# georghess/neurad-studio

Hardware: NVIDIA H100
Metric: rays/sec (camera+lidar) (higher is better)
Workload: dtype f32

## Files before the change

### neurad-studio_b200/csrc/b200nerf.cu

```cuda
#include <cuda_runtime.h>

#include <cstdio>
#include <cstring>
#include <new>
#include <string>
#include <vector>

#include "../../include/b200nerf.h"
#include "nff_device.h"
#include "nff_lane.h"
#include "rgb_decoder.cuh"
#include "modules.cuh"

using namespace nff;

static thread_local std::string g_err;
static int fail(int code, const std::string& msg) {
  g_err = msg;
  return code;
}
#define CUDA_TRY(expr)                                                                                   \
  do {                                                                                                   \
    cudaError_t e_ = (expr);                                                                             \
    if (e_ != cudaSuccess)                                                                               \
// ... 56 lines not shown
    if (prev != dev) cudaSetDevice(dev);
  }
  ~DeviceGuard() { cudaSetDevice(prev); }
};

int make_grid(const b200nerf_grid_desc* d, const float* table, Grid* g) {
  REQUIRE(d != nullptr, "grid descriptor is NULL");
  REQUIRE(d->num_levels >= 1 && d->num_levels <= kMaxLevels, "num_levels must be in [1,16]");
  REQUIRE(d->log2_hashmap_size >= 1 && d->log2_hashmap_size <= 30, "log2_hashmap_size out of range");
  g->table = table;
  g->T = 1u << d->log2_hashmap_size;
  g->mask = g->T - 1u;
  g->L = d->num_levels;
  g->F = d->features_per_level;
  for (int i = 0; i < kMaxLevels; ++i) g->res[i] = i < d->num_levels ? d->scalings[i] : 0.f;
  return 0;
}
}

#ifndef NFF_WARPS
#define NFF_WARPS 8
#endif
constexpr int kSmemMaxOptIn = 227 * 1024;
constexpr int kRenderWarps = NFF_WARPS;

template <int WARPS>
__global__ void __launch_bounds__(WARPS * 32, 16 / WARPS) nff_render_kernel(const __grid_constant__ RenderParams P) {
  extern __shared__ __align__(16) unsigned char smem_raw[];
  float* mlp_s = reinterpret_cast<float*>(smem_raw);
  constexpr int kMlpBytes = (kMainMlpFloats * 4 + 15) / 16 * 16;
// ... 60 lines not shown
  *ray_out = active ? ray : fallback;
  return active;
}

__device__ __forceinline__ int64_t lane_patches(const RenderParams& P) {
  return P.rays.image_width > 0 ? lane_units(P) * (kLaneThreads / 32) : (P.n_rays + 31) / 32;
}
__device__ __forceinline__ bool lane_patch_ray(const RenderParams& P, int64_t patch, int lane_, int64_t* ray_out) {
  constexpr int kPatchesPerUnit = kLaneThreads / 32;
  return lane_unit_ray(P, patch / kPatchesPerUnit, (int)(patch % kPatchesPerUnit) * 32 + lane_, ray_out);
}

#ifndef NFF_SAMPLE_CTAS
#define NFF_SAMPLE_CTAS 2
#endif
template <int LAYOUT>
__global__ void __launch_bounds__(kLaneThreads, NFF_SAMPLE_CTAS) nff_sample_lane_kernel(const __grid_constant__ RenderParams P,
                                                                                        float* __restrict__ scratch,
                                                                                        float* __restrict__ handoff) {
  const int tid = threadIdx.x, warp = __shfl_sync(0xffffffffu, (int)(threadIdx.x >> 5), 0), lane_ = tid & 31;
  const LaneScratch sc = lane_scratch_of(scratch, blockIdx.x);
  constexpr int kPPU = kLaneThreads / 32;
  const int64_t n_patches = lane_patches(P);
  const int64_t full_rounds = n_patches / kPPU / gridDim.x;
  const int64_t r0 = full_rounds * gridDim.x * kPPU, rest = n_patches - r0;
  const int64_t p0 = r0 + rest * blockIdx.x / gridDim.x, p1 = r0 + rest * (blockIdx.x + 1) / gridDim.x;
  for (int64_t it = 0;; ++it) {
    int64_t patch;
    if (it < full_rounds) {
      patch = (it * gridDim.x + blockIdx.x) * kPPU + warp;
    } else {
      patch = p0 + warp + (it - full_rounds) * kPPU;
      if (patch >= p1) break;
    }
    int64_t ray;
    const bool active = lane_patch_ray(P, patch, lane_, &ray);
    const LaneRay R = lane_ray_setup(P, sc, tid, ray);
    float* col = active ? handoff + ray : sc.bins2 + tid;
    sample_ray_lane<LAYOUT>(P, sc, R, tid, ray, active, col, active ? P.n_rays : (int64_t)kLaneThreads);
  }
}

template <int LAYOUT>
__global__ void __launch_bounds__(kLaneThreads, kLaneCtasPerSm) nff_shade_lane_kernel(const __grid_constant__ RenderParams P,
                                                                                      float* __restrict__ scratch,
                                                                                      const float* __restrict__ handoff) {
  extern __shared__ __align__(128) unsigned char smem_shade[];
  TcShared* tcs = reinterpret_cast<TcShared*>(smem_shade);
  const int tid = threadIdx.x, warp = __shfl_sync(0xffffffffu, (int)(threadIdx.x >> 5), 0), group = warp >> 2;
  tc_stage_weights(*tcs, P.main_mlp_nn, tid, kLaneThreads, true);
  tc::fence_async_smem();
  __syncthreads();
  MlpLaneTc mlp;
  mlp.t = tcs;
// ... 711 lines not shown
  c->sm_count = prop.multiProcessorCount;
  CUDA_TRY(cudaFuncSetAttribute(nff_render_kernel<kRenderWarps>, cudaFuncAttributeMaxDynamicSharedMemorySize,
                                (int)((kMainMlpFloats * 4 + 15) / 16 * 16 + kRenderWarps * sizeof(WarpShared))));
  CUDA_TRY(cudaFuncSetAttribute(nff_render_tc_kernel<kRenderWarps>, cudaFuncAttributeMaxDynamicSharedMemorySize,
                                (int)(tc_smem_bytes(kRenderWarps * 32) + kRenderWarps * sizeof(WarpSharedTc))));
  CUDA_TRY(cudaMalloc((void**)&c->d_status, sizeof(int)));
  CUDA_TRY(cudaMemset(c->d_status, 0, sizeof(int)));
  CUDA_TRY(cudaFuncSetAttribute(nff_render_lane_kernel, cudaFuncAttributeMaxDynamicSharedMemorySize,
                                (int)lane_tc_smem_bytes()));
  c->lane_ctas = c->sm_count * (kLaneCtasPerSm > NFF_SAMPLE_CTAS ? kLaneCtasPerSm : NFF_SAMPLE_CTAS);
  CUDA_TRY(cudaMalloc((void**)&c->d_lane_scratch, sizeof(float) * lane_scratch_floats_per_cta() * c->lane_ctas));
  CUDA_TRY(cudaFuncSetAttribute(nff_shade_lane_kernel<0>, cudaFuncAttributeMaxDynamicSharedMemorySize,
                                (int)lane_tc_smem_bytes()));
  CUDA_TRY(cudaFuncSetAttribute(nff_shade_lane_kernel<1>, cudaFuncAttributeMaxDynamicSharedMemorySize,
                                (int)lane_tc_smem_bytes()));
  CUDA_TRY(cudaFuncSetAttribute(nff_sample_lane_kernel<0>, cudaFuncAttributePreferredSharedMemoryCarveout, 0));
  CUDA_TRY(cudaFuncSetAttribute(nff_sample_lane_kernel<1>, cudaFuncAttributePreferredSharedMemoryCarveout, 0));
  CUDA_TRY(cudaMalloc((void**)&c->d_minmax, 2 * sizeof(unsigned)));
  c->handoff_rays = (int64_t)1 << 21;
  CUDA_TRY(cudaMalloc((void**)&c->d_handoff, sizeof(float) * (kS2 + 1) * c->handoff_rays));
  CUDA_TRY(cudaMalloc((void**)&c->d_grad_actor_ptrs, sizeof(float*) * kModMaxActors));
  *out = c;
  return 0;
}

int b200nerf_destroy(b200nerf_ctx* c) {
  if (!c) return 0;
  DeviceGuard g(c->device);
  for (int i = 0; i < 3; ++i) {
    cudaFree((void*)c->d_actor_tables[i]);
    cudaFree(c->d_decoder[i]);
  }
// ... 36 lines not shown
    return fail(B200NERF_ERR_UNSUPPORTED,
                "fused kernel is specialised for NeuRAD's grid shapes (main: 8 levels x 4 features, proposal: 6 x 1)");
  if (n_actors > 0) {
    REQUIRE(ad && atabs_host, "actor grid descriptor / tables missing");
    if (int e = make_grid(ad, nullptr, &fg.act)) return e;
    if (fg.act.L != 4 || fg.act.F != wantF)
      return fail(B200NERF_ERR_UNSUPPORTED, "actor grids must have 4 levels and the static grid's feature width");
    cudaFree((void*)c->d_actor_tables[field]);
    c->d_actor_tables[field] = nullptr;
    CUDA_TRY(cudaMalloc((void**)&c->d_actor_tables[field], sizeof(float*) * n_actors));
    CUDA_TRY(cudaMemcpy((void*)c->d_actor_tables[field], atabs_host, sizeof(float*) * n_actors, cudaMemcpyHostToDevice));
    fg.actor_tables = c->d_actor_tables[field];
  }
  fg.static_scale = static_scale;
  fg.actor_scale = actor_scale;
  fg.decoder = c->d_decoder[field];
  c->fields[field] = fg;
  c->have_field[field] = true;
  c->field_layout[field] = 0;
  if (field == B200NERF_FIELD_MAIN) c->layout = 0;
  return 0;
}

namespace {
int make_tcnn_grid(const b200nerf_tcnn_grid_desc* d, const float* params, int want_dims, Grid* g) {
  REQUIRE(d != nullptr && params != nullptr, "tcnn grid descriptor / parameters are NULL");
  REQUIRE(d->num_levels >= 1 && d->num_levels <= kMaxLevels, "num_levels must be in [1,16]");
  REQUIRE(d->n_input_dims == want_dims, "tcnn grid has the wrong number of input dimensions (static: 3, actors: 4)");
  *g = Grid{};
  g->table = params;
// ... 26 lines not shown
  DeviceGuard g(c->device);
  FieldGrids fg{};
  if (int e = make_tcnn_grid(sd, sparams, 3, &fg.stat)) return e;
  const int wantL = field == B200NERF_FIELD_MAIN ? 8 : 6, wantF = field == B200NERF_FIELD_MAIN ? 4 : 1;
  if (fg.stat.L != wantL || fg.stat.F != wantF)
    return fail(B200NERF_ERR_UNSUPPORTED,
                "fused kernel is specialised for NeuRAD's grid shapes (main: 8 levels x 4 features, proposal: 6 x 1)");
  if (n_actors > 0) {
    if (int e = make_tcnn_grid(ad, aparams, 4, &fg.act)) return e;
    if (fg.act.L != 4 || fg.act.F != wantF)
      return fail(B200NERF_ERR_UNSUPPORTED, "the 4-D actor grid must have 4 levels and the static grid's feature width");
  }
  fg.n_actors_f = (float)(n_actors > 0 ? n_actors : 1);
  fg.static_scale = static_scale;
  fg.actor_scale = actor_scale;
  fg.decoder = c->d_decoder[field];
  c->fields[field] = fg;
  c->have_field[field] = true;
  c->field_layout[field] = 1;
  if (field == B200NERF_FIELD_MAIN) c->layout = 1;
  return 0;
}

int b200nerf_set_proposal_decoder(b200nerf_ctx* c, int field, const float* weight, int in_dim) {
  REQUIRE(c, "ctx is NULL");
  REQUIRE(field == B200NERF_FIELD_PROP0 || field == B200NERF_FIELD_PROP1, "decoder belongs to a proposal field");
  REQUIRE(weight && in_dim == 6, "density_decoder must be Linear(6, 1)");
  DeviceGuard g(c->device);
  if (!c->d_decoder[field]) CUDA_TRY(cudaMalloc((void**)&c->d_decoder[field], sizeof(float) * 8));
  CUDA_TRY(cudaMemcpyAsync(c->d_decoder[field], weight, sizeof(float) * in_dim, cudaMemcpyDeviceToDevice, c->param_stream));
// ... 117 lines not shown
            "density_field_of_round entries must name a proposal field");
  DeviceGuard g(c->device);
  if (!c->d_u1) CUDA_TRY(cudaMalloc((void**)&c->d_u1, sizeof(float) * (kS1 + 1)));
  if (!c->d_u2) CUDA_TRY(cudaMalloc((void**)&c->d_u2, sizeof(float) * (kS2 + 1)));
  CUDA_TRY(cudaMemcpy(c->d_u1, u1_host, sizeof(float) * (kS1 + 1), cudaMemcpyHostToDevice));
  CUDA_TRY(cudaMemcpy(c->d_u2, u2_host, sizeof(float) * (kS2 + 1), cudaMemcpyHostToDevice));
  Sampling s{};
  s.lam = lam;
  s.scaling = scaling;
  s.sky_distance = sky;
  s.hist_pad = hist_pad;
  s.cam_area_scale = camera_area_scale;
  double lam1 = lam - 1.0 < 0 ? -(lam - 1.0) : (lam - 1.0);
  s.lam_1 = (float)lam1;
  s.ratio = (float)(lam1 / (double)lam);
  s.u1 = c->d_u1;
  s.u2 = c->d_u2;
  s.field_of_round[0] = field_of_round[0];
  s.field_of_round[1] = field_of_round[1];
  c->samp = s;
  c->n_prop0 = n_prop0; c->n_prop1 = n_prop1; c->n_nerf = n_nerf;
  c->have_samp = true;
  return 0;
}

int b200nerf_nff_render_fwd(b200nerf_ctx* c, const b200nerf_rays* rays, int64_t n_rays, const b200nerf_outputs* out,
                            const b200nerf_trace* trace, void* stream) {
  REQUIRE(c && rays && out, "NULL argument");
  REQUIRE(n_rays >= 0, "negative ray count");
  REQUIRE(rays->image_width >= 0, "negative image_width");
// ... 61 lines not shown
    }
    const int fdim = kNff + c->app.dim;
    for (int64_t start = 0; start < n_rays; start += slice) {
      const int64_t cnt = n_rays - start < slice ? n_rays - start : slice;
      RenderParams Q = P;
      Q.n_rays = cnt;
      offset_rays(Q, start, fdim);
      int64_t need = (cnt + kLaneThreads - 1) / kLaneThreads;
      if (rays->image_width > 0) {
        const int64_t W = rays->image_width, H = (cnt + W - 1) / W;
        need = ((W + 31) / 32) * ((H + kLaneThreads / 32 - 1) / (kLaneThreads / 32));
      }
      const int64_t max_a = (int64_t)c->sm_count * NFF_SAMPLE_CTAS, max_b = (int64_t)c->sm_count * kLaneCtasPerSm;
      const int64_t patches = rays->image_width > 0 ? need * (kLaneThreads / 32) : (cnt + 31) / 32, groups = (patches + 3) / 4;
      const int64_t grid_a = patches < max_a ? patches : max_a, grid_b = groups < max_b ? groups : max_b;
      if (c->layout == 1) {
        nff_sample_lane_kernel<1><<<(int)grid_a, kLaneThreads, 0, st>>>(Q, c->d_lane_scratch, c->d_handoff);
        nff_shade_lane_kernel<1><<<(int)grid_b, kLaneThreads, smem, st>>>(Q, c->d_lane_scratch, c->d_handoff);
      } else {
        nff_sample_lane_kernel<0><<<(int)grid_a, kLaneThreads, 0, st>>>(Q, c->d_lane_scratch, c->d_handoff);
        nff_shade_lane_kernel<0><<<(int)grid_b, kLaneThreads, smem, st>>>(Q, c->d_lane_scratch, c->d_handoff);
      }
    }
  } else if (c->mlp_mode == 2) {
    const size_t smem = lane_tc_smem_bytes();
    int64_t need = (n_rays + kLaneThreads - 1) / kLaneThreads;
    if (rays->image_width > 0) {
      const int64_t W = rays->image_width, H = (n_rays + W - 1) / W;
      need = ((W + 31) / 32) * ((H + kLaneThreads / 32 - 1) / (kLaneThreads / 32));
    }
    int lane_blocks = (int)(need < c->lane_ctas ? need : c->lane_ctas);
    nff_render_lane_kernel<<<lane_blocks, kLaneThreads, smem, st>>>(P, c->d_lane_scratch);
  } else if (c->mlp_mode == 1) {
    const size_t smem = tc_smem_bytes(WARPS * 32) + WARPS * sizeof(WarpSharedTc);
    nff_render_tc_kernel<WARPS><<<blocks, WARPS * 32, smem, st>>>(P);
// ... 83 lines not shown
  CUDA_TRY(cudaGetLastError());
  return 0;
}

static int make_spacing(int kind, float power_lambda, float power_scaling, SpacingArgs* a) {
  REQUIRE(kind >= B200NERF_SPACING_UNIFORM && kind <= B200NERF_SPACING_LOG, "unknown spacing kind");
  a->kind = kind;
  if (kind == B200NERF_SPACING_POWER) {
    REQUIRE(power_lambda != 0.f && power_lambda != 1.f, "power_lambda 0 / 1 (log / identity spacing) is not supported");
    REQUIRE(power_scaling > 0.f, "power_scaling must be positive");
    a->power.lam = power_lambda;
    a->power.scaling = power_scaling;
    double lam1 = power_lambda - 1.0 < 0 ? -(power_lambda - 1.0) : (power_lambda - 1.0);
    a->power.lam_1 = (float)lam1;
    a->power.ratio = (float)(lam1 / (double)power_lambda);
  }
  return 0;
}

int b200nerf_spaced_sample(b200nerf_ctx* c, int kind, float power_lambda, float power_scaling, const float* nears,
                           const float* fars, int64_t n_rays, int n_samples, float* bins_s, float* bins_e, void* stream) {
  REQUIRE(c, "ctx is NULL");
  REQUIRE(n_rays >= 0 && n_samples >= 1, "bad sample grid");
  if (n_rays == 0) return 0;
  REQUIRE(fars && bins_e, "NULL argument");
  SpacingArgs a{};
  if (int rc = make_spacing(kind, power_lambda, power_scaling, &a)) return rc;
  DeviceGuard g(c->device);
  const int64_t n = n_rays * (n_samples + 1);
  spaced_sample_kernel<<<(unsigned)((n + 255) / 256), 256, 0, (cudaStream_t)stream>>>(a, nears, fars, n_rays, n_samples, bins_s, bins_e);
// ... 801 lines not shown
```

### neurad-studio_b200/csrc/nff_device.h

```cpp
#pragma once
#include "nff_params.h"
#include "simt.h"

#ifndef NFF_G_PROP
#define NFF_G_PROP 1
#endif
#ifndef NFF_G_ACT
#define NFF_G_ACT 2
#endif
#ifndef NFF_ILP
#define NFF_ILP 2
#endif
#ifndef NFF_F4_UNROLL
#define NFF_F4_UNROLL 2
#endif
#ifndef NFF_FAST_RCP
#define NFF_FAST_RCP 1
#endif
#ifndef NFF_PARITY_STD
#define NFF_PARITY_STD 0
#endif
#ifndef NFF_PARITY_LERP
#define NFF_PARITY_LERP 0
#endif
// ... 20 lines not shown
  for (int d = 1; d < 32; d <<= 1) {
    float n = shfl_up(v, d);
    if (lane() >= d) v += n;
  }
  return v;
}
NFF_D float warp_scan_mul(float v) {
#pragma unroll
  for (int d = 1; d < 32; d <<= 1) {
    float n = shfl_up(v, d);
    if (lane() >= d) v *= n;
  }
  return v;
}

NFF_D float pow_lam(float t, float e) { return e == -1.0f ? frcp(t) : powf(t, e); }
NFF_D float spacing_fn(float x, const Sampling& s) {
  float t = fadd(fdiv(fmul(x, s.scaling), s.lam_1), 1.0f);
  return fmul(s.ratio, fsub(pow_lam(t, s.lam), 1.0f));
}
NFF_D float spacing_fn_inv(float y, const Sampling& s) {
  float t = fadd(fdiv(fmul(y, s.lam), s.lam_1), 1.0f);
  t = fmaxf(t, 1e-10f);
  float r = fmul(fsub(pow_lam(t, s.lam == -1.0f ? -1.0f : 1.0f / s.lam), 1.0f), s.lam_1);
  return fdiv(r, s.scaling);
}
NFF_D float to_euclid(float u, float s_near, float s_far, const Sampling& s) {
  return spacing_fn_inv(fadd(fmul(u, s_far), fmul(fsub(1.0f, u), s_near)), s);
}
NFF_D float linspace01(int i, int n) {
  float step = fdiv(1.0f, (float)n);
  return i < (n + 1) / 2 ? fmul(step, (float)i) : fsub(1.0f, fmul(step, (float)(n - i)));
}

struct Gauss {
  float x, y, z, std;
};
NFF_D Gauss sample_gaussian(const float o[3], const float d[3], float area, float start, float end) {
  float md = fdiv(fsub(end, start), 2.0f);
  float t = fadd(start, md);
  Gauss g;
  g.x = fadd(o[0], fmul(d[0], t));
  g.y = fadd(o[1], fmul(d[1], t));
  g.z = fadd(o[2], fmul(d[2], t));
  float cs = fmul(area, fmul(t, t));
#if NFF_PARITY_STD
  g.std = powf(fmul(cs, md), 0.33333334f);
#else
  g.std = cbrtf(fmul(cs, md));
#endif
  return g;
}
NFF_D Gauss contract(Gauss g, float scale) {
  float x = fdiv(g.x, scale), y = fdiv(g.y, scale), z = fdiv(g.z, scale);
#if NFF_PARITY_STD
  float sd = fdiv(g.std, scale);
#else
  float sd = fmul(g.std, frcp(scale));
#endif
  float mag = fmaxf(fmaxf(fabsf(x), fabsf(y)), fabsf(z));
  if (!(mag < 1.0f)) {
    const float a = fsub(2.0f, frcp(mag));
    x = fmul(a, fdiv(x, mag));
    y = fmul(a, fdiv(y, mag));
    z = fmul(a, fdiv(z, mag));
#if NFF_PARITY_STD
    float q = fdiv(powf(fsub(fmul(2.0f, mag), 1.0f), 0.33333334f), mag);
#else
    float q = fmul(cbrtf(fsub(fmul(2.0f, mag), 1.0f)), frcp(mag));
#endif
    sd = fmul(sd, fmul(q, q));
  }
  Gauss r;
  r.x = fmul(fadd(x, 2.0f), 0.25f);
  r.y = fmul(fadd(y, 2.0f), 0.25f);
  r.z = fmul(fadd(z, 2.0f), 0.25f);
  r.std = fmul(sd, 0.25f);
  return r;
}

struct Cell {
  uint32_t hx[2], hy[2], hz[2];
  float ox, oy, oz;
};
NFF_D Cell grid_cell(float x, float y, float z, float res) {
  float px = fmul(x, res), py = fmul(y, res), pz = fmul(z, res);
  float fx = floorf(px), fy = floorf(py), fz = floorf(pz);
  Cell c;
  const uint32_t ix = (uint32_t)(int32_t)fx, iy = (uint32_t)(int32_t)fy, iz = (uint32_t)(int32_t)fz;
  c.hx[0] = ix;
  c.hx[1] = ix + (px != fx ? 1u : 0u);
  c.hy[0] = iy * 2654435761u;
  c.hy[1] = (iy + (py != fy ? 1u : 0u)) * 2654435761u;
// ... 57 lines not shown
  float ox, oy, oz;
};
template <int SH>
NFF_D CellB<SH> grid_cell_b(float x, float y, float z, float res) {
  const float px = fmul(x, res), py = fmul(y, res), pz = fmul(z, res);
  const float fx = floorf(px), fy = floorf(py), fz = floorf(pz);
  CellB<SH> c;
  c.hx = (uint32_t)(int32_t)fx << SH;
  c.hy = (uint32_t)(int32_t)fy * (2654435761u << SH);
  c.hz = (uint32_t)(int32_t)fz * (805459861u << SH);
  c.ox = fsub(px, fx);
  c.oy = fsub(py, fy);
  c.oz = fsub(pz, fz);
  return c;
}
NFF_D uint32_t xor_and(uint32_t a, uint32_t b, uint32_t m) {
#if defined(__CUDACC__)
  uint32_t d;
  asm("lop3.b32 %0, %1, %2, %3, 0x28;" : "=r"(d) : "r"(a), "r"(b), "r"(m));
  return d;
#else
  return (a ^ b) & m;
#endif
}
template <int SH>
NFF_D void cell_offsets_b(const CellB<SH>& c, uint32_t maskb, uint32_t r[8]) {
  const uint32_t hx1 = c.hx + (1u << SH), hy1 = c.hy + (2654435761u << SH), hz1 = c.hz + (805459861u << SH);
  const uint32_t a11 = hy1 ^ hz1, a01 = c.hy ^ hz1, a10 = hy1 ^ c.hz, a00 = c.hy ^ c.hz;
  r[0] = xor_and(hx1, a11, maskb);
  r[1] = xor_and(hx1, a01, maskb);
// ... 31 lines not shown
  float f4756 = blend_f(f47, c.oy, f56, iy);
  return blend_f(f0312, c.oz, f4756, iz);
}

template <int L, int G>
NFF_D float encode_f1_dot(const float* NFF_RESTRICT table, const Grid& gr, Gauss g, const float* NFF_RESTRICT dec) {
  static_assert(L % G == 0, "group size must divide the level count");
  float acc = 0.0f;
  const uint32_t maskb = gr.mask << 2;
#pragma unroll
  for (int l0 = 0; l0 < L; l0 += G) {
    CellB<2> c[G];
    float f[G][8];
#pragma unroll
    for (int j = 0; j < G; ++j) {
      c[j] = grid_cell_b<2>(g.x, g.y, g.z, gr.res[l0 + j]);
      uint32_t r[8];
      cell_offsets_b<2>(c[j], maskb, r);
      const char* base = level_base(table, l0 + j, gr.T, 4);
#pragma unroll
      for (int k = 0; k < 8; ++k) f[j][k] = ldg_at<float>(base, r[k]);
    }
#pragma unroll
    for (int j = 0; j < G; ++j) {
      float w = level_weight(gr.res[l0 + j], g.std);
      float v = trilerp_b<2>(f[j], c[j], 1.0f - c[j].ox, 1.0f - c[j].oy, 1.0f - c[j].oz);
      acc = fmaf(fmul(v, w), ldg(dec + l0 + j), acc);
    }
  }
  return acc;
}
// ... 685 lines not shown
```

### neurad-studio_b200/csrc/nff_lane.h

```cpp
#pragma once
#include "nff_device.h"

namespace nff {

#ifndef NFF_LANE_THREADS
#define NFF_LANE_THREADS 512
#endif
#ifndef NFF_F4_WEIGHTS
#define NFF_F4_WEIGHTS 0
#endif
constexpr int kLaneThreads = NFF_LANE_THREADS;
constexpr int kLaneCtasPerSm = 512 / kLaneThreads;
constexpr int kCandFloats = 16;
constexpr int kLaneMaxCand = 32;

struct LaneScratch {
  float* w;
  float* bins1;
  float* bins2;
  float* cand;
};
NFF_HD size_t lane_scratch_floats_per_cta() {
  return (size_t)kLaneThreads * (kS0 + (kS1 + 1) + (kS2 + 1) + kLaneMaxCand * kCandFloats);
}
// ... 81 lines not shown
#pragma unroll
      for (int i = 0; i < 12; ++i) M_out[i] = M[i];
    }
  }
  return hit;
}

template <int LAYOUT = 0>
NFF_D float lane_proposal_density(const FieldGrids& fg, const LaneScratch& sc, int tid, int n_cand, const Gauss& g,
                                  int* actor_id) {
  float pb[3], M[12];
  int a = n_cand > 0 ? lane_actor_of_sample(sc, tid, n_cand, g, pb, M) : -1;
  float acc;
  if (a >= 0) {
    Gauss ga = {pb[0], pb[1], pb[2], g.std};
    ga = contract(ga, fg.actor_scale);
    if (LAYOUT == 1) {
      const float x4[4] = {ga.x, ga.y, ga.z, fdiv((float)a, fg.n_actors_f)};
      acc = tcnn_encode_f1_dot<4>(fg.act, 4, x4, ga.std, fg.decoder);
    } else {
      acc = encode_f1_dot<4, NFF_G_ACT>(fg.actor_tables[a], fg.act, ga, fg.decoder);
    }
  } else {
    Gauss gs = contract(g, fg.static_scale);
    if (LAYOUT == 1) {
      const float x3[3] = {gs.x, gs.y, gs.z};
      acc = tcnn_encode_f1_dot<3>(fg.stat, 6, x3, gs.std, fg.decoder);
    } else {
      acc = encode_f1_dot<6, NFF_G_PROP>(fg.stat.table, fg.stat, gs, fg.decoder);
    }
  }
  *actor_id = a;
  return expf(acc);
}

NFF_D void encode_f4_col(const float* NFF_RESTRICT table, const Grid& gr, int L, Gauss g, float* x , int pitch) {
  const uint32_t maskb = gr.mask << 4;
#pragma unroll 2
  for (int l = 0; l < L; ++l) {
// ... 40 lines not shown
#endif
  }
}

struct LaneRoundIO {
  int S, S_new;
  const float* u_tab;
  float* bins_out;
  int64_t bins_stride;
  float* tr_w;
  int32_t* tr_aid;
  float* tr_bins_s;
  float* tr_bins_e;
  int32_t* tr_inds;
};
template <int LAYOUT = 0>
NFF_D float lane_proposal_round(const RenderParams& P, const FieldGrids& fg, const LaneScratch& sc, int tid, int n_cand,
                                const LaneRoundIO& io, const float* bins_in, const float o[3], const float d[3], float area,
                                float s_near, float s_far, int64_t ray) {
  const Sampling& sp = P.samp;
  const int S = io.S, S_new = io.S_new;
  auto edge = [bins_in, S](int i) { return bins_in ? bins_in[(size_t)i * kLaneThreads] : linspace01(i, S); };
  double excl = 0.0, tot_d = 0.0;
  float depth_acc = 0.0f;
  float e_prev = to_euclid(edge(0), s_near, s_far, sp);
#pragma unroll 1
  for (int s = 0; s < S; ++s) {
    const float T = expf(-(float)excl);
    float w = 0.0f;
    if (!(vote_all_converged(T == 0.0f) && io.tr_aid == nullptr)) {
      const float e0 = e_prev;
      const float e1 = to_euclid(edge(s + 1), s_near, s_far, sp);
      e_prev = e1;
      Gauss g = sample_gaussian(o, d, area, e0, e1);
      int aid;
      float dens = lane_proposal_density<LAYOUT>(fg, sc, tid, n_cand, g, &aid);
      float dd = fmul(fsub(e1, e0), dens);
      float alpha = fsub(1.0f, expf(-dd));
      excl += (double)dd;
      w = nan_to_num(fmul(alpha, T));
      depth_acc = fadd(depth_acc, fmul(w, fmul(fadd(e0, e1), 0.5f)));
      if (io.tr_aid) io.tr_aid[ray * S + s] = aid;
    }
    if (io.tr_w) io.tr_w[ray * S + s] = w;
    w = fadd(w, sp.hist_pad);
    sc.w[(size_t)s * kLaneThreads + tid] = w;
    tot_d += (double)w;
  }
  float tot = (float)tot_d;
  const float padding = fmaxf(fsub(1e-5f, tot), 0.0f);
  const float pad_each = fdiv(padding, (float)S);
  tot = fadd(tot, padding);
  int k = 1;
  double run = (double)fdiv(fadd(sc.w[tid], pad_each), tot);
  float c_km1 = 0.0f, c_k = fminf(1.0f, (float)run);
  float w_next = sc.w[(size_t)kLaneThreads + tid];
#pragma unroll 1
  for (int i = 0; i <= S_new; ++i) {
    const float u = ldg(io.u_tab + i);
    while (k <= S && c_k <= u) {
      ++k;
      c_km1 = c_k;
      if (k <= S) {
        const float wk = w_next;
        w_next = sc.w[(size_t)(k < S ? k : S - 1) * kLaneThreads + tid];
        run += (double)fdiv(fadd(wk, pad_each), tot);
        c_k = fminf(1.0f, (float)run);
      }
    }
    const int above = k > S ? S : k;
    const float b0 = edge(k - 1), b1 = edge(above);
    float t = nan_to_num(fdiv(fsub(u, c_km1), fsub(k > S ? c_km1 : c_k, c_km1)));
    t = fminf(fmaxf(t, 0.0f), 1.0f);
    const float nb = fadd(b0, fmul(t, fsub(b1, b0)));
    io.bins_out[(size_t)i * io.bins_stride] = nb;
    if (io.tr_inds) io.tr_inds[ray * (S_new + 1) + i] = k;
    if (io.tr_bins_s) io.tr_bins_s[ray * (S_new + 1) + i] = nb;
    if (io.tr_bins_e) io.tr_bins_e[ray * (S_new + 1) + i] = to_euclid(nb, s_near, s_far, sp);
  }
  return depth_acc;
}

struct MlpLaneFfma {
  static constexpr int kPitch = kLaneThreads;
  const float* w;
  float* panel_;
  int sh_tcnn = 0;
  NFF_D float* panel() const { return panel_; }
  NFF_D void run(const float* x, const float dir[3], float& sdf, float* feat, int ) const {
    float h[kHidden], go[kNff + 1], in2[kNff + kSh], h2[kHidden];
    dense<kGeoIn, kHidden, kHidden, true>(w + kOffGeoW0, w + kOffGeoB0, x, h);
    dense<kHidden, kNff + 1, kGeoOutP, false>(w + kOffGeoW1, w + kOffGeoB1, h, go);
    sdf = go[0];
// ... 170 lines not shown
  R.area = fmul(ldg(P.rays.pixel_area + ray), lidar ? 1.0f : sp.cam_area_scale);
  R.time = ldg(P.rays.times + ray);
  float far_ = P.rays.fars ? ldg(P.rays.fars + ray) : 1.0e6f;
  far_ = fminf(far_, sp.sky_distance);
  const float near_ = P.rays.nears ? ldg(P.rays.nears + ray) : 0.0f;
  R.s_near = spacing_fn(near_, sp);
  R.s_far = spacing_fn(far_, sp);
  int overflow = 0;
  R.n_cand = lane_actor_candidates(P.actors, R.time, R.o, R.d, sc, tid, &overflow);
#if defined(__CUDACC__)
  if (overflow && P.status) atomicExch(P.status, 3);
#endif
  return R;
}

template <int LAYOUT = 0>
NFF_D void sample_ray_lane(const RenderParams& P, const LaneScratch& sc, const LaneRay& R, int tid, int64_t ray, bool active,
                           float* bins2, int64_t bins2_stride) {
  const Sampling& sp = P.samp;
  float prop_depth[2];
#pragma unroll 1
  for (int rd = 0; rd < 2; ++rd) {
    LaneRoundIO io;
    io.S = rd == 0 ? kS0 : kS1;
    io.S_new = rd == 0 ? kS1 : kS2;
    io.u_tab = rd == 0 ? sp.u1 : sp.u2;
    io.bins_out = rd == 0 ? sc.bins1 + tid : bins2;
    io.bins_stride = rd == 0 ? (int64_t)kLaneThreads : bins2_stride;
    io.tr_w = !active ? nullptr : rd == 0 ? P.trace.prop_weights_0 : P.trace.prop_weights_1;
    io.tr_aid = !active ? nullptr : rd == 0 ? P.trace.actor_id_0 : P.trace.actor_id_1;
    io.tr_bins_s = !active ? nullptr : rd == 0 ? P.trace.bins_s_1 : P.trace.bins_s_2;
    io.tr_bins_e = !active ? nullptr : rd == 0 ? P.trace.bins_e_1 : P.trace.bins_e_2;
    io.tr_inds = !active ? nullptr : rd == 0 ? P.trace.inds_1 : P.trace.inds_2;
    prop_depth[rd] = lane_proposal_round<LAYOUT>(P, P.fields[sp.field_of_round[rd]], sc, tid, R.n_cand, io,
                                         rd == 0 ? nullptr : sc.bins1 + tid, R.o, R.d, R.area, R.s_near, R.s_far, ray);
  }
  if (active) {
    P.out.prop_depth_0[ray] = prop_depth[0];
    P.out.prop_depth_1[ray] = prop_depth[1];
  }
}

template <class Mlp, int LAYOUT = 0>
NFF_D void shade_ray_lane(const RenderParams& P, const LaneScratch& sc, const LaneRay& R, Mlp& mlp, int tid, int64_t ray,
                          bool active, const float* bins2, int64_t bins2_stride) {
  const Sampling& sp = P.samp;
  const float* o = R.o;
  const float* d = R.d;
  const float area = R.area, time = R.time, s_near = R.s_near, s_far = R.s_far;
// ... 160 lines not shown
```

### neurad-studio_b200/csrc/nff_params.h

```cpp
#pragma once
#include <stdint.h>

#include "../../include/b200nerf.h"

namespace nff {

constexpr int kMaxLevels = 16;
constexpr int kMaxCand = 16;
constexpr int kS0 = 128;
constexpr int kS1 = 64;
constexpr int kS2 = 32;
constexpr int kGeoIn = 32;
constexpr int kHidden = 32;
constexpr int kNff = 32;
constexpr int kSh = 16;
constexpr int kApp = 16;
constexpr int kFeatOut = 64;

constexpr int kGeoOutP = 36;
constexpr int kOffGeoW0 = 0;
constexpr int kOffGeoB0 = kOffGeoW0 + kGeoIn * kHidden;
constexpr int kOffGeoW1 = kOffGeoB0 + kHidden;
constexpr int kOffGeoB1 = kOffGeoW1 + kHidden * kGeoOutP;
constexpr int kOffFeatW0 = kOffGeoB1 + kGeoOutP;
// ... 12 lines not shown
constexpr int kOffLidB2 = kOffLidW2 + kHidden * kLidOutP;
constexpr int kLidarMlpFloats = kOffLidB2 + kLidOutP;

constexpr int kNnGeoW0 = 0;
constexpr int kNnGeoB0 = kNnGeoW0 + kHidden * kGeoIn;
constexpr int kNnGeoW1 = kNnGeoB0 + kHidden;
constexpr int kNnGeoB1 = kNnGeoW1 + (kNff + 1) * kHidden;
constexpr int kNnFeatW0 = kNnGeoB1 + (kNff + 1);
constexpr int kNnFeatB0 = kNnFeatW0 + kHidden * (kNff + kSh);
constexpr int kNnFeatW1 = kNnFeatB0 + kHidden;
constexpr int kNnFeatB1 = kNnFeatW1 + kHidden * kHidden;
constexpr int kNnFeatW2 = kNnFeatB1 + kHidden;
constexpr int kNnFeatB2 = kNnFeatW2 + kNff * kHidden;
constexpr int kNnMlpFloats = kNnFeatB2 + kNff;

struct Grid {
  const float* table;
  uint32_t mask;
  uint32_t T;
  int32_t L, F;
  float res[kMaxLevels];
  float pos_scale[kMaxLevels];
  uint32_t lvl_res[kMaxLevels];
  uint32_t lvl_off[kMaxLevels];
  uint32_t lvl_mask[kMaxLevels];
  uint32_t dense_bits;
  int32_t n_dims;
};

struct FieldGrids {
  Grid stat;
  Grid act;
  const float* const* actor_tables;
  float static_scale, actor_scale;
  float n_actors_f;
  const float* decoder;
};

struct Actors {
  int32_t n_actors, n_times;
  const float* times;
  const float* keyframes;
  const uint8_t* present;
  const float* bounds;
  const float* radii;
};

struct Sampling {
  float lam, scaling, sky_distance, hist_pad, cam_area_scale;
  float lam_1, ratio;
  const float* u1;
  const float* u2;
  int32_t field_of_round[2];
};

struct Appearance {
  const float* emb;
  int32_t num_embeds, dim, eps;
  float duration;
};

struct RenderParams {
  FieldGrids fields[3];
  const float* main_mlp;
  const float* main_mlp_nn;
  const float* lidar_mlp;
  int* status;
  float beta;
// ... 14 lines not shown
```

Baseline: 78.38 million.

## Speed up sampling kernel with precomputed divisors, fast floor, and trace specialization

```diff
diff --git a/neurad-studio_b200/csrc/b200nerf.cu b/neurad-studio_b200/csrc/b200nerf.cu
--- a/neurad-studio_b200/csrc/b200nerf.cu
+++ b/neurad-studio_b200/csrc/b200nerf.cu
@@ -94,6 +94,8 @@
   g->L = d->num_levels;
   g->F = d->features_per_level;
   for (int i = 0; i < kMaxLevels; ++i) g->res[i] = i < d->num_levels ? d->scalings[i] : 0.f;
+  for (int i = 0; i < d->num_levels; ++i)
+    REQUIRE(!std::signbit(d->scalings[i]) && d->scalings[i] < 4194304.0f, "grid resolutions must lie in [+0, 2^22)");
   return 0;
 }
 }
@@ -184,7 +186,7 @@
 #ifndef NFF_SAMPLE_CTAS
 #define NFF_SAMPLE_CTAS 2
 #endif
-template <int LAYOUT>
+template <int LAYOUT, bool TRACE>
 __global__ void __launch_bounds__(kLaneThreads, NFF_SAMPLE_CTAS) nff_sample_lane_kernel(const __grid_constant__ RenderParams P,
                                                                                         float* __restrict__ scratch,
                                                                                         float* __restrict__ handoff) {
@@ -207,7 +209,7 @@
     const bool active = lane_patch_ray(P, patch, lane_, &ray);
     const LaneRay R = lane_ray_setup(P, sc, tid, ray);
     float* col = active ? handoff + ray : sc.bins2 + tid;
-    sample_ray_lane<LAYOUT>(P, sc, R, tid, ray, active, col, active ? P.n_rays : (int64_t)kLaneThreads);
+    sample_ray_lane<LAYOUT, TRACE>(P, sc, R, tid, ray, active, col, active ? P.n_rays : (int64_t)kLaneThreads);
   }
 }
 
@@ -949,8 +951,10 @@
                                 (int)lane_tc_smem_bytes()));
   CUDA_TRY(cudaFuncSetAttribute(nff_shade_lane_kernel<1>, cudaFuncAttributeMaxDynamicSharedMemorySize,
                                 (int)lane_tc_smem_bytes()));
-  CUDA_TRY(cudaFuncSetAttribute(nff_sample_lane_kernel<0>, cudaFuncAttributePreferredSharedMemoryCarveout, 0));
-  CUDA_TRY(cudaFuncSetAttribute(nff_sample_lane_kernel<1>, cudaFuncAttributePreferredSharedMemoryCarveout, 0));
+  CUDA_TRY(cudaFuncSetAttribute(nff_sample_lane_kernel<0, false>, cudaFuncAttributePreferredSharedMemoryCarveout, 0));
+  CUDA_TRY(cudaFuncSetAttribute(nff_sample_lane_kernel<1, false>, cudaFuncAttributePreferredSharedMemoryCarveout, 0));
+  CUDA_TRY(cudaFuncSetAttribute(nff_sample_lane_kernel<0, true>, cudaFuncAttributePreferredSharedMemoryCarveout, 0));
+  CUDA_TRY(cudaFuncSetAttribute(nff_sample_lane_kernel<1, true>, cudaFuncAttributePreferredSharedMemoryCarveout, 0));
   CUDA_TRY(cudaMalloc((void**)&c->d_minmax, 2 * sizeof(unsigned)));
   c->handoff_rays = (int64_t)1 << 21;
   CUDA_TRY(cudaMalloc((void**)&c->d_handoff, sizeof(float) * (kS2 + 1) * c->handoff_rays));
@@ -1017,6 +1021,8 @@
   }
   fg.static_scale = static_scale;
   fg.actor_scale = actor_scale;
+  fg.div_static = divisor_of(static_scale);
+  fg.div_actor = divisor_of(actor_scale);
   fg.decoder = c->d_decoder[field];
   c->fields[field] = fg;
   c->have_field[field] = true;
@@ -1073,6 +1079,8 @@
   fg.n_actors_f = (float)(n_actors > 0 ? n_actors : 1);
   fg.static_scale = static_scale;
   fg.actor_scale = actor_scale;
+  fg.div_static = divisor_of(static_scale);
+  fg.div_actor = divisor_of(actor_scale);
   fg.decoder = c->d_decoder[field];
   c->fields[field] = fg;
   c->have_field[field] = true;
@@ -1220,6 +1228,8 @@
   double lam1 = lam - 1.0 < 0 ? -(lam - 1.0) : (lam - 1.0);
   s.lam_1 = (float)lam1;
   s.ratio = (float)(lam1 / (double)lam);
+  s.div_lam_1 = divisor_of(s.lam_1);
+  s.div_scaling = divisor_of(s.scaling);
   s.u1 = c->d_u1;
   s.u2 = c->d_u2;
   s.field_of_round[0] = field_of_round[0];
@@ -1311,11 +1321,15 @@
       const int64_t max_a = (int64_t)c->sm_count * NFF_SAMPLE_CTAS, max_b = (int64_t)c->sm_count * kLaneCtasPerSm;
       const int64_t patches = rays->image_width > 0 ? need * (kLaneThreads / 32) : (cnt + 31) / 32, groups = (patches + 3) / 4;
       const int64_t grid_a = patches < max_a ? patches : max_a, grid_b = groups < max_b ? groups : max_b;
+      const b200nerf_trace& tr = Q.trace;
+      const bool trace_sampling = tr.prop_weights_0 || tr.prop_weights_1 || tr.actor_id_0 || tr.actor_id_1 || tr.bins_s_1 ||
+                                  tr.bins_s_2 || tr.bins_e_1 || tr.bins_e_2 || tr.inds_1 || tr.inds_2;
+      auto sample_kernel = c->layout == 1 ? (trace_sampling ? nff_sample_lane_kernel<1, true> : nff_sample_lane_kernel<1, false>)
+                                          : (trace_sampling ? nff_sample_lane_kernel<0, true> : nff_sample_lane_kernel<0, false>);
+      sample_kernel<<<(int)grid_a, kLaneThreads, 0, st>>>(Q, c->d_lane_scratch, c->d_handoff);
       if (c->layout == 1) {
-        nff_sample_lane_kernel<1><<<(int)grid_a, kLaneThreads, 0, st>>>(Q, c->d_lane_scratch, c->d_handoff);
         nff_shade_lane_kernel<1><<<(int)grid_b, kLaneThreads, smem, st>>>(Q, c->d_lane_scratch, c->d_handoff);
       } else {
-        nff_sample_lane_kernel<0><<<(int)grid_a, kLaneThreads, 0, st>>>(Q, c->d_lane_scratch, c->d_handoff);
         nff_shade_lane_kernel<0><<<(int)grid_b, kLaneThreads, smem, st>>>(Q, c->d_lane_scratch, c->d_handoff);
       }
     }
@@ -1429,6 +1443,8 @@
     double lam1 = power_lambda - 1.0 < 0 ? -(power_lambda - 1.0) : (power_lambda - 1.0);
     a->power.lam_1 = (float)lam1;
     a->power.ratio = (float)(lam1 / (double)power_lambda);
+    a->power.div_lam_1 = divisor_of(a->power.lam_1);
+    a->power.div_scaling = divisor_of(a->power.scaling);
   }
   return 0;
 }
diff --git a/neurad-studio_b200/csrc/nff_device.h b/neurad-studio_b200/csrc/nff_device.h
--- a/neurad-studio_b200/csrc/nff_device.h
+++ b/neurad-studio_b200/csrc/nff_device.h
@@ -58,30 +58,66 @@
   return v;
 }
 
-NFF_D float pow_lam(float t, float e) { return e == -1.0f ? frcp(t) : powf(t, e); }
+NFF_HD Divisor divisor_of(float b, float y) {
+  uint32_t u;
+  std::memcpy(&u, &b, 4);
+  const int eb = (int)((u >> 23) & 0xffu);
+  Divisor d;
+  d.y = y;
+  d.lo = 0u;
+  d.span = 0u;
+  if (eb >= 1 && eb <= 252) {
+    const int lo = eb - 100 > 32 ? eb - 100 : 32, hi = eb + 100 < 254 ? eb + 100 : 254;
+    d.lo = (uint32_t)lo << 23;
+    d.span = ((uint32_t)(hi + 1) << 23) - d.lo;
+  }
+  return d;
+}
+NFF_HD Divisor divisor_of(float b) { return divisor_of(b, 1.0f / b); }
+NFF_D float div_by(float a, float b, const Divisor& d) {
+#if defined(__CUDACC__)
+  if ((__float_as_uint(a) & 0x7fffffffu) - d.lo < d.span) {
+    const float q0 = __fmul_rn(a, d.y);
+    const float r = __fmaf_rn(-b, q0, a);
+    return __fmaf_rn(d.y, r, q0);
+  }
+  return __fdiv_rn(a, b);
+#else
+  (void)d;
+  return a / b;
+#endif
+}
+NFF_D Divisor divisor_dev(float b) { return divisor_of(b, frcp(b)); }
+
+#if defined(__CUDACC__)
+__device__ __noinline__ float pow_general(float t, float e) { return powf(t, e); }
+#else
+inline float pow_general(float t, float e) { return powf(t, e); }
+#endif
+NFF_D float pow_lam(float t, float e) { return e == -1.0f ? frcp(t) : pow_general(t, e); }
 NFF_D float spacing_fn(float x, const Sampling& s) {
   float t = fadd(fdiv(fmul(x, s.scaling), s.lam_1), 1.0f);
   return fmul(s.ratio, fsub(pow_lam(t, s.lam), 1.0f));
 }
 NFF_D float spacing_fn_inv(float y, const Sampling& s) {
-  float t = fadd(fdiv(fmul(y, s.lam), s.lam_1), 1.0f);
+  float t = fadd(div_by(fmul(y, s.lam), s.lam_1, s.div_lam_1), 1.0f);
   t = fmaxf(t, 1e-10f);
   float r = fmul(fsub(pow_lam(t, s.lam == -1.0f ? -1.0f : 1.0f / s.lam), 1.0f), s.lam_1);
-  return fdiv(r, s.scaling);
+  return div_by(r, s.scaling, s.div_scaling);
 }
 NFF_D float to_euclid(float u, float s_near, float s_far, const Sampling& s) {
   return spacing_fn_inv(fadd(fmul(u, s_far), fmul(fsub(1.0f, u), s_near)), s);
 }
-NFF_D float linspace01(int i, int n) {
-  float step = fdiv(1.0f, (float)n);
+NFF_D float linspace01_step(int i, int n, float step) {
   return i < (n + 1) / 2 ? fmul(step, (float)i) : fsub(1.0f, fmul(step, (float)(n - i)));
 }
+NFF_D float linspace01(int i, int n) { return linspace01_step(i, n, fdiv(1.0f, (float)n)); }
 
 struct Gauss {
   float x, y, z, std;
 };
 NFF_D Gauss sample_gaussian(const float o[3], const float d[3], float area, float start, float end) {
-  float md = fdiv(fsub(end, start), 2.0f);
+  float md = fmul(fsub(end, start), 0.5f);
   float t = fadd(start, md);
   Gauss g;
   g.x = fadd(o[0], fmul(d[0], t));
@@ -95,23 +131,19 @@
 #endif
   return g;
 }
-NFF_D Gauss contract(Gauss g, float scale) {
-  float x = fdiv(g.x, scale), y = fdiv(g.y, scale), z = fdiv(g.z, scale);
-#if NFF_PARITY_STD
-  float sd = fdiv(g.std, scale);
-#else
-  float sd = fmul(g.std, frcp(scale));
-#endif
+NFF_D Gauss contract_scaled(float x, float y, float z, float sd) {
   float mag = fmaxf(fmaxf(fabsf(x), fabsf(y)), fabsf(z));
   if (!(mag < 1.0f)) {
-    const float a = fsub(2.0f, frcp(mag));
-    x = fmul(a, fdiv(x, mag));
-    y = fmul(a, fdiv(y, mag));
-    z = fmul(a, fdiv(z, mag));
+    const float rm = frcp(mag);
+    const Divisor dm = divisor_of(mag, rm);
+    const float a = fsub(2.0f, rm);
+    x = fmul(a, div_by(x, mag, dm));
+    y = fmul(a, div_by(y, mag, dm));
+    z = fmul(a, div_by(z, mag, dm));
 #if NFF_PARITY_STD
-    float q = fdiv(powf(fsub(fmul(2.0f, mag), 1.0f), 0.33333334f), mag);
+    float q = div_by(powf(fsub(fmul(2.0f, mag), 1.0f), 0.33333334f), mag, dm);
 #else
-    float q = fmul(cbrtf(fsub(fmul(2.0f, mag), 1.0f)), frcp(mag));
+    float q = fmul(cbrtf(fsub(fmul(2.0f, mag), 1.0f)), rm);
 #endif
     sd = fmul(sd, fmul(q, q));
   }
@@ -121,6 +153,24 @@
   r.z = fmul(fadd(z, 2.0f), 0.25f);
   r.std = fmul(sd, 0.25f);
   return r;
+}
+NFF_D Gauss contract(Gauss g, float scale) {
+#if NFF_PARITY_STD
+  const float sd = fdiv(g.std, scale);
+#else
+  const float sd = fmul(g.std, frcp(scale));
+#endif
+  return contract_scaled(fdiv(g.x, scale), fdiv(g.y, scale), fdiv(g.z, scale), sd);
+}
+NFF_D Gauss contract(Gauss g, float scale, const Divisor& ds) {
+#if NFF_PARITY_STD
+  const float sd = div_by(g.std, scale, ds);
+#elif defined(__CUDACC__)
+  const float sd = fmul(g.std, ds.y);
+#else
+  const float sd = fmul(g.std, frcp(scale));
+#endif
+  return contract_scaled(div_by(g.x, scale, ds), div_by(g.y, scale, ds), div_by(g.z, scale, ds), sd);
 }
 
 struct Cell {
@@ -208,6 +258,32 @@
   c.oz = fsub(pz, fz);
   return c;
 }
+struct Floor22 {
+  float f;
+  int32_t i;
+};
+NFF_D Floor22 floor22(float p) {
+#if defined(__CUDACC__)
+  const float t = __fadd_rd(p, 12582912.0f);
+  return Floor22{__fsub_rn(t, 12582912.0f), __float_as_int(t) - 0x4B400000};
+#else
+  const float f = floorf(p);
+  return Floor22{f, (int32_t)f};
+#endif
+}
+template <int SH>
+NFF_D CellB<SH> grid_cell_unit(float x, float y, float z, float res) {
+  const float px = fmul(x, res), py = fmul(y, res), pz = fmul(z, res);
+  const Floor22 fx = floor22(px), fy = floor22(py), fz = floor22(pz);
+  CellB<SH> c;
+  c.hx = (uint32_t)fx.i << SH;
+  c.hy = (uint32_t)fy.i * (2654435761u << SH);
+  c.hz = (uint32_t)fz.i * (805459861u << SH);
+  c.ox = fsub(px, fx.f);
+  c.oy = fsub(py, fy.f);
+  c.oz = fsub(pz, fz.f);
+  return c;
+}
 NFF_D uint32_t xor_and(uint32_t a, uint32_t b, uint32_t m) {
 #if defined(__CUDACC__)
   uint32_t d;
@@ -269,7 +345,7 @@
     float f[G][8];
 #pragma unroll
     for (int j = 0; j < G; ++j) {
-      c[j] = grid_cell_b<2>(g.x, g.y, g.z, gr.res[l0 + j]);
+      c[j] = grid_cell_unit<2>(g.x, g.y, g.z, gr.res[l0 + j]);
       uint32_t r[8];
       cell_offsets_b<2>(c[j], maskb, r);
       const char* base = level_base(table, l0 + j, gr.T, 4);
diff --git a/neurad-studio_b200/csrc/nff_lane.h b/neurad-studio_b200/csrc/nff_lane.h
--- a/neurad-studio_b200/csrc/nff_lane.h
+++ b/neurad-studio_b200/csrc/nff_lane.h
@@ -119,7 +119,7 @@
   float acc;
   if (a >= 0) {
     Gauss ga = {pb[0], pb[1], pb[2], g.std};
-    ga = contract(ga, fg.actor_scale);
+    ga = contract(ga, fg.actor_scale, fg.div_actor);
     if (LAYOUT == 1) {
       const float x4[4] = {ga.x, ga.y, ga.z, fdiv((float)a, fg.n_actors_f)};
       acc = tcnn_encode_f1_dot<4>(fg.act, 4, x4, ga.std, fg.decoder);
@@ -127,7 +127,7 @@
       acc = encode_f1_dot<4, NFF_G_ACT>(fg.actor_tables[a], fg.act, ga, fg.decoder);
     }
   } else {
-    Gauss gs = contract(g, fg.static_scale);
+    Gauss gs = contract(g, fg.static_scale, fg.div_static);
     if (LAYOUT == 1) {
       const float x3[3] = {gs.x, gs.y, gs.z};
       acc = tcnn_encode_f1_dot<3>(fg.stat, 6, x3, gs.std, fg.decoder);
@@ -198,13 +198,19 @@
   float* tr_bins_e;
   int32_t* tr_inds;
 };
-template <int LAYOUT = 0>
+template <int LAYOUT = 0, bool TRACE = true>
 NFF_D float lane_proposal_round(const RenderParams& P, const FieldGrids& fg, const LaneScratch& sc, int tid, int n_cand,
                                 const LaneRoundIO& io, const float* bins_in, const float o[3], const float d[3], float area,
                                 float s_near, float s_far, int64_t ray) {
   const Sampling& sp = P.samp;
   const int S = io.S, S_new = io.S_new;
-  auto edge = [bins_in, S](int i) { return bins_in ? bins_in[(size_t)i * kLaneThreads] : linspace01(i, S); };
+  float* const tr_w = TRACE ? io.tr_w : nullptr;
+  int32_t* const tr_aid = TRACE ? io.tr_aid : nullptr;
+  float* const tr_bins_s = TRACE ? io.tr_bins_s : nullptr;
+  float* const tr_bins_e = TRACE ? io.tr_bins_e : nullptr;
+  int32_t* const tr_inds = TRACE ? io.tr_inds : nullptr;
+  const float step = fdiv(1.0f, (float)S);
+  auto edge = [bins_in, S, step](int i) { return bins_in ? bins_in[(size_t)i * kLaneThreads] : linspace01_step(i, S, step); };
   double excl = 0.0, tot_d = 0.0;
   float depth_acc = 0.0f;
   float e_prev = to_euclid(edge(0), s_near, s_far, sp);
@@ -212,7 +218,7 @@
   for (int s = 0; s < S; ++s) {
     const float T = expf(-(float)excl);
     float w = 0.0f;
-    if (!(vote_all_converged(T == 0.0f) && io.tr_aid == nullptr)) {
+    if (!(vote_all_converged(T == 0.0f) && tr_aid == nullptr)) {
       const float e0 = e_prev;
       const float e1 = to_euclid(edge(s + 1), s_near, s_far, sp);
       e_prev = e1;
@@ -224,9 +230,9 @@
       excl += (double)dd;
       w = nan_to_num(fmul(alpha, T));
       depth_acc = fadd(depth_acc, fmul(w, fmul(fadd(e0, e1), 0.5f)));
-      if (io.tr_aid) io.tr_aid[ray * S + s] = aid;
-    }
-    if (io.tr_w) io.tr_w[ray * S + s] = w;
+      if (tr_aid) tr_aid[ray * S + s] = aid;
+    }
+    if (tr_w) tr_w[ray * S + s] = w;
     w = fadd(w, sp.hist_pad);
     sc.w[(size_t)s * kLaneThreads + tid] = w;
     tot_d += (double)w;
@@ -235,8 +241,9 @@
   const float padding = fmaxf(fsub(1e-5f, tot), 0.0f);
   const float pad_each = fdiv(padding, (float)S);
   tot = fadd(tot, padding);
+  const Divisor dtot = divisor_dev(tot);
   int k = 1;
-  double run = (double)fdiv(fadd(sc.w[tid], pad_each), tot);
+  double run = (double)div_by(fadd(sc.w[tid], pad_each), tot, dtot);
   float c_km1 = 0.0f, c_k = fminf(1.0f, (float)run);
   float w_next = sc.w[(size_t)kLaneThreads + tid];
 #pragma unroll 1
@@ -248,7 +255,7 @@
       if (k <= S) {
         const float wk = w_next;
         w_next = sc.w[(size_t)(k < S ? k : S - 1) * kLaneThreads + tid];
-        run += (double)fdiv(fadd(wk, pad_each), tot);
+        run += (double)div_by(fadd(wk, pad_each), tot, dtot);
         c_k = fminf(1.0f, (float)run);
       }
     }
@@ -258,9 +265,9 @@
     t = fminf(fmaxf(t, 0.0f), 1.0f);
     const float nb = fadd(b0, fmul(t, fsub(b1, b0)));
     io.bins_out[(size_t)i * io.bins_stride] = nb;
-    if (io.tr_inds) io.tr_inds[ray * (S_new + 1) + i] = k;
-    if (io.tr_bins_s) io.tr_bins_s[ray * (S_new + 1) + i] = nb;
-    if (io.tr_bins_e) io.tr_bins_e[ray * (S_new + 1) + i] = to_euclid(nb, s_near, s_far, sp);
+    if (tr_inds) tr_inds[ray * (S_new + 1) + i] = k;
+    if (tr_bins_s) tr_bins_s[ray * (S_new + 1) + i] = nb;
+    if (tr_bins_e) tr_bins_e[ray * (S_new + 1) + i] = to_euclid(nb, s_near, s_far, sp);
   }
   return depth_acc;
 }
@@ -461,7 +468,7 @@
   return R;
 }
 
-template <int LAYOUT = 0>
+template <int LAYOUT = 0, bool TRACE = true>
 NFF_D void sample_ray_lane(const RenderParams& P, const LaneScratch& sc, const LaneRay& R, int tid, int64_t ray, bool active,
                            float* bins2, int64_t bins2_stride) {
   const Sampling& sp = P.samp;
@@ -474,12 +481,12 @@
     io.u_tab = rd == 0 ? sp.u1 : sp.u2;
     io.bins_out = rd == 0 ? sc.bins1 + tid : bins2;
     io.bins_stride = rd == 0 ? (int64_t)kLaneThreads : bins2_stride;
-    io.tr_w = !active ? nullptr : rd == 0 ? P.trace.prop_weights_0 : P.trace.prop_weights_1;
-    io.tr_aid = !active ? nullptr : rd == 0 ? P.trace.actor_id_0 : P.trace.actor_id_1;
-    io.tr_bins_s = !active ? nullptr : rd == 0 ? P.trace.bins_s_1 : P.trace.bins_s_2;
-    io.tr_bins_e = !active ? nullptr : rd == 0 ? P.trace.bins_e_1 : P.trace.bins_e_2;
-    io.tr_inds = !active ? nullptr : rd == 0 ? P.trace.inds_1 : P.trace.inds_2;
-    prop_depth[rd] = lane_proposal_round<LAYOUT>(P, P.fields[sp.field_of_round[rd]], sc, tid, R.n_cand, io,
+    io.tr_w = !active || !TRACE ? nullptr : rd == 0 ? P.trace.prop_weights_0 : P.trace.prop_weights_1;
+    io.tr_aid = !active || !TRACE ? nullptr : rd == 0 ? P.trace.actor_id_0 : P.trace.actor_id_1;
+    io.tr_bins_s = !active || !TRACE ? nullptr : rd == 0 ? P.trace.bins_s_1 : P.trace.bins_s_2;
+    io.tr_bins_e = !active || !TRACE ? nullptr : rd == 0 ? P.trace.bins_e_1 : P.trace.bins_e_2;
+    io.tr_inds = !active || !TRACE ? nullptr : rd == 0 ? P.trace.inds_1 : P.trace.inds_2;
+    prop_depth[rd] = lane_proposal_round<LAYOUT, TRACE>(P, P.fields[sp.field_of_round[rd]], sc, tid, R.n_cand, io,
                                          rd == 0 ? nullptr : sc.bins1 + tid, R.o, R.d, R.area, R.s_near, R.s_far, ray);
   }
   if (active) {
diff --git a/neurad-studio_b200/csrc/nff_params.h b/neurad-studio_b200/csrc/nff_params.h
--- a/neurad-studio_b200/csrc/nff_params.h
+++ b/neurad-studio_b200/csrc/nff_params.h
@@ -50,6 +50,11 @@
 constexpr int kNnFeatB2 = kNnFeatW2 + kNff * kHidden;
 constexpr int kNnMlpFloats = kNnFeatB2 + kNff;
 
+struct Divisor {
+  float y;
+  uint32_t lo, span;
+};
+
 struct Grid {
   const float* table;
   uint32_t mask;
@@ -69,6 +74,7 @@
   Grid act;
   const float* const* actor_tables;
   float static_scale, actor_scale;
+  Divisor div_static, div_actor;
   float n_actors_f;
   const float* decoder;
 };
@@ -88,6 +94,7 @@
   const float* u1;
   const float* u2;
   int32_t field_of_round[2];
+  Divisor div_lam_1, div_scaling;
 };
 
 struct Appearance {
```

Result: faster. 79.35 million, median of 6 (+1.2%).
